# PeterFWS/Structure-PLP-SLAM

Measured on AMD Instinct MI355X. Metric: frames/sec ORB+LSD extract+match, 640x480 TUM-RGBD, 1/2/4/8 GPU, higher is better.
Workload: dtype u8

## Files before the change

include/plp_front.h:

```cpp
#ifndef PLP_FRONT_H
#define PLP_FRONT_H

#include <stddef.h>
#include <stdint.h>

#ifdef __cplusplus
extern "C" {
#endif

typedef enum plp_status {
    PLP_OK = 0,
    PLP_ERR_INVALID_ARG = 1,
    PLP_ERR_NO_DEVICE = 2,
    PLP_ERR_HIP = 3,
    PLP_ERR_CAPACITY = 4,
    PLP_ERR_OVERFLOW = 5,
    PLP_ERR_UNSUPPORTED = 6
} plp_status;

const char* plp_strerror(plp_status s);
const char* plp_last_error(void);
int plp_version(void);
int plp_device_count(void);

// ... 85 lines not shown

plp_status plp_line_extract(plp_line* ctx, const uint8_t* img, int32_t rows, int32_t cols, size_t step,
                            plp_keyline* kl, uint8_t* lbd, double* linefn, int32_t cap, int32_t* n_out);
plp_status plp_line_extract_batch_device(plp_line* ctx, const uint8_t* d_imgs, int32_t B, int32_t rows, int32_t cols,
                                         size_t step, size_t frame_stride, plp_keyline* d_kl, uint8_t* d_lbd,
                                         double* d_linefn, int32_t cap, int32_t* d_counts, void* hip_stream);
plp_status plp_line_last_batch_status(plp_line* ctx);
plp_status plp_line_set_profiling(plp_line* ctx, int32_t enable);
plp_status plp_line_get_stage_times(plp_line* ctx, double* ms9, int64_t* n_batches);
plp_status plp_line_set_grow_waves(plp_line* ctx, int32_t waves);
typedef enum plp_seed_order { PLP_SEED_ORDER_STABLE = 0, PLP_SEED_ORDER_LIBSTDCXX = 1 } plp_seed_order;
plp_status plp_line_set_seed_order(plp_line* ctx, int32_t order);
plp_status plp_line_get_seed_order(const plp_line* ctx, int32_t* order);
plp_status plp_line_trim(plp_line* ctx);

typedef enum plp_line_debug_id { PLP_LINE_DBG_SCALED = 0, PLP_LINE_DBG_ORDER = 1, PLP_LINE_DBG_RAW = 2, PLP_LINE_DBG_ALL_KL = 3,
                                 PLP_LINE_DBG_ALL_LBD = 4, PLP_LINE_DBG_SOBEL_DX = 5, PLP_LINE_DBG_SOBEL_DY = 6,
                                 PLP_LINE_DBG_GROW_STATS = 7  } plp_line_debug_id;
plp_status plp_line_debug_read(plp_line* ctx, plp_line_debug_id what, int32_t frame, void* dst, size_t dst_bytes, int64_t* n_out);
int32_t plp_model_index_sort_host(const int32_t* sizes, int32_t n, int32_t depth_limit, uint32_t* idx);
int32_t plp_model_quadtree_rank_sort_host(const uint32_t* keys, int32_t n, int32_t shift, uint32_t* perm);
int32_t plp_model_seed_introsort_host(uint32_t* entries, int64_t n, int32_t depth_limit, uint32_t skip_key);
plp_status plp_seed_introsort_debug(int32_t device, uint32_t* entries, int64_t n, int32_t depth_limit, uint32_t skip_key, int32_t variant, int32_t* n_live);
int32_t plp_model_sincos_host(const float* a, int64_t n, float* c, float* s, uint8_t* proven);
int32_t plp_model_null_vector4_host(const double* A, int32_t n, double* out_v, int32_t* out_sweeps);
plp_status plp_line_scaled_size(const plp_line* ctx, int32_t* rows, int32_t* cols);
plp_status plp_line_debug_grow_profile(plp_line* ctx, int64_t* out12);

typedef struct plp_keyline plp_keyline_fwd_;
typedef struct plp_matcher plp_matcher;
plp_status plp_matcher_create(int device, plp_matcher** out);
void plp_matcher_destroy(plp_matcher* ctx);

typedef enum plp_match_mode {
    PLP_MATCH_MODE_LANDMARKS = 0,
    PLP_MATCH_MODE_LAST_FRAME = 1,
    PLP_MATCH_MODE_BRUTE_FORCE = 2,
    PLP_MATCH_MODE_LANDMARKS_LINE = 3,
    PLP_MATCH_MODE_LAST_FRAME_LINE = 4,
    PLP_MATCH_MODE_BOW = 5,
    PLP_MATCH_MODE_FUSE = 6,
    PLP_MATCH_MODE_FUSE_LINE = 7,
    PLP_MATCH_MODE_TRIANGULATION = 8
} plp_match_mode;

#define PLP_MATCH_FLAG_NO_CHI2 1
// ... 1294 lines not shown
```

structure-plp-slam_amd/__init__.py:

```python
import ctypes as C
import math
import os
import pathlib
import subprocess

import numpy as np

from ._core import (LIB_PATH, PLP_ERR_CAPACITY, PLP_ERR_HIP, PLP_ERR_INVALID_ARG, PLP_ERR_NO_DEVICE, PLP_ERR_OVERFLOW, PLP_ERR_UNSUPPORTED, PLP_OK, PlpError,
                    ROOT, _API, _I32, _PKG, _SZ, _VP, _check, _lib, _p, api_symbols, build, lib)
from ._abi import *
from ._abi import _struct
from ._global_ba import (GLOBAL_BA_OUTPUTS, LOOP_BA_PROPAGATE_OUTPUTS, _chol_dense, _global_ba_host, _global_ba_kw, _loop_ba_propagate_host, global_bundle_adjuster,
                         loop_bundle_adjuster, model_chol_dense, model_global_ba, model_loop_ba_propagate)
from ._essential import (ESSENTIAL_OUTPUTS, _essential_ransac_host, essential_solver, model_essential_check, model_essential_draw, model_essential_fit,
                         model_essential_ransac)
from ._two_view import (TWO_VIEW_OUTPUTS, _two_view_pose_host, bearing_vector_initializer, model_check_pose, model_essential_decompose, model_two_view_pose,
                        two_view_args)
from ._line_update import (CORRECT_LINE_ERASED, CORRECT_LINE_NO_REF, CORRECT_LINE_NO_VERTEX, CORRECT_LINE_OK, LINE_MOVE_OUTPUTS, TRIM_DEPTH_POSITIVE, TRIM_INDEX_RANGE,
                           TRIM_MAX_CHANGE, TRIM_MAX_CHANGE_THR, TRIM_NO_REF, TRIM_NOT_OBSERVED, TRIM_OK, TRIM_OUTPUTS, TRIM_REJECTED, TRIM_SKIPPED,
                           correct_landmark_lines_args_c, line_update_entries, loop_ba_propagate_lines_args_c, model_correct_landmark_lines,
                           model_loop_ba_propagate_lines, model_trim_line_endpoints, trim_line_endpoints_args_c)
from ._marshal import _rows_u8, array_or_none, dev_ptr, dev_ptrs, host_ptr, host_ptrs, model_call, model_draw, out_arrays, set_outputs, stream_handle, wanted


# ... 2 lines not shown
    out = np.zeros(max(len(xys), 1), np.int32)
    m = lib().plp_model_quadtree_host(_p(xys), len(xys), level_w, level_h, quota, _p(out))
    return out[:m].copy()


def model_quadtree_rank_sort(keys, shift=0):
    k = np.ascontiguousarray(keys, np.uint32)
    perm = np.zeros(max(len(k), 1), np.uint32)
    assert lib().plp_model_quadtree_rank_sort_host(_p(k), len(k), int(shift), _p(perm)) == len(k)
    return perm[:len(k)].copy()


def model_seed_introsort(entries, depth_limit=-1, skip_key=0):
    e = np.ascontiguousarray(entries, np.uint32).copy()
    assert lib().plp_model_seed_introsort_host(_p(e), e.size, int(depth_limit), int(skip_key)) == 0
    return e


def seed_introsort_debug(entries, depth_limit=-1, skip_key=0, variant=0, device=0, return_live=False):
    e = np.ascontiguousarray(entries, np.uint32).copy()
    nl = C.c_int32(e.size)
    _check(lib().plp_seed_introsort_debug(int(device), _p(e), e.size, int(depth_limit), int(skip_key), int(variant), C.byref(nl)))
    return (e, nl.value) if return_live else e


def model_index_sort(sizes, depth_limit=-1):
    sz = np.ascontiguousarray(sizes, np.int32)
    idx = np.zeros(len(sz), np.uint32)
    assert lib().plp_model_index_sort_host(_p(sz), len(sz), int(depth_limit), _p(idx)) == len(sz)
    return idx


def model_sincos(a):
    a = np.ascontiguousarray(a, np.float32)
    c = np.zeros(a.shape, np.float32); s = np.zeros(a.shape, np.float32); ok = np.zeros(a.shape, np.uint8)
    lib().plp_model_sincos_host(_p(a), a.size, _p(c), _p(s), _p(ok))
    return c, s, ok.astype(bool)


def _landmark_geometry_host(call, lines, pose, feats, pos_w, ref_kf, obs_offsets, obs_kf, obs_idx, scale_factors, scale_factors_lsd, skip, counts,
                            out):
    po = np.ascontiguousarray(pose, np.float64).reshape(-1, 15)
    F = len(po)
    ft = np.ascontiguousarray(feats, KL_DTYPE if lines else KP_DTYPE).reshape(F, -1)
    M = ft.shape[1]
    pw = np.ascontiguousarray(pos_w, np.float64).reshape(-1, 6 if lines else 3)
# ... 2906 lines not shown
```

structure-plp-slam_amd/_core.py:

```python

import ctypes as C
import os
import pathlib
import subprocess


_PKG = pathlib.Path(__file__).resolve().parent
ROOT = _PKG.parent
LIB_PATH = pathlib.Path(os.environ["PLP_FRONT_LIB"]).resolve() if os.environ.get("PLP_FRONT_LIB") else _PKG / "libplp_front.so"


PLP_OK, PLP_ERR_INVALID_ARG, PLP_ERR_NO_DEVICE, PLP_ERR_HIP, PLP_ERR_CAPACITY, PLP_ERR_OVERFLOW, PLP_ERR_UNSUPPORTED = range(7)


class PlpError(RuntimeError):
    def __init__(self, status, detail):
        super().__init__(f"plp_front status {status}: {detail}")
        self.status = status


def build(verbose=False):
    r = subprocess.run(["make", "-j", str(min(8, os.cpu_count() or 1)), "-C", str(_PKG / "csrc")], capture_output=not verbose, text=True)
    if r.returncode != 0:
        raise RuntimeError("building libplp_front.so failed:\n" + (r.stdout or "") + (r.stderr or ""))
# ... 19 lines not shown
    ("plp_orb_last_batch_status", C.c_int, [_VP]),
    ("plp_orb_set_profiling", C.c_int, [_VP, _I32]),
    ("plp_orb_get_stage_times", C.c_int, [_VP, _VP, _VP]),
    ("plp_orb_pyramid_level_size", C.c_int, [_VP, _I32, _VP, _VP]),
    ("plp_orb_pyramid_host", C.c_int, [_VP, _I32, _I32, _VP, _SZ]),
    ("plp_orb_debug_read", C.c_int, [_VP, C.c_int, _I32, _I32, _VP, _SZ, _VP]),
    ("plp_model_quadtree_host", _I32, [_VP, _I32, _I32, _I32, C.c_uint32, _VP]),
    ("plp_model_quadtree_rank_sort_host", _I32, [_VP, _I32, _I32, _VP]),
    ("plp_model_sincos_host", _I32, [_VP, C.c_int64, _VP, _VP, _VP]),
    ("plp_model_index_sort_host", _I32, [_VP, _I32, _I32, _VP]),
    ("plp_model_null_vector4_host", _I32, [_VP, _I32, _VP, _VP]),
    ("plp_line_create", C.c_int, [C.c_int, _VP]),
    ("plp_line_destroy", None, [_VP]),
    ("plp_line_extract", C.c_int, [_VP, _VP, _I32, _I32, _SZ, _VP, _VP, _VP, _I32, _VP]),
    ("plp_line_extract_batch_device", C.c_int, [_VP, _VP, _I32, _I32, _I32, _SZ, _SZ, _VP, _VP, _VP, _I32, _VP, _VP]),
    ("plp_line_last_batch_status", C.c_int, [_VP]),
    ("plp_line_set_profiling", C.c_int, [_VP, _I32]),
    ("plp_line_set_grow_waves", C.c_int, [_VP, _I32]),
    ("plp_line_set_seed_order", C.c_int, [_VP, _I32]),
    ("plp_line_get_seed_order", C.c_int, [_VP, _VP]),
    ("plp_line_trim", C.c_int, [_VP]),
    ("plp_model_seed_introsort_host", _I32, [_VP, C.c_int64, _I32, C.c_uint32]),
    ("plp_seed_introsort_debug", C.c_int, [_I32, _VP, C.c_int64, _I32, C.c_uint32, _I32, _VP]),
    ("plp_line_get_stage_times", C.c_int, [_VP, _VP, _VP]),
    ("plp_line_debug_read", C.c_int, [_VP, C.c_int, _I32, _VP, _SZ, _VP]),
    ("plp_line_scaled_size", C.c_int, [_VP, _VP, _VP]),
    ("plp_line_debug_grow_profile", C.c_int, [_VP, _VP]),
    ("plp_matcher_create", C.c_int, [C.c_int, _VP]),
    ("plp_matcher_destroy", None, [_VP]),
    ("plp_match_device", C.c_int, [_VP, _VP, _VP]),
    ("plp_match_host", C.c_int, [_VP, _VP]),
    ("plp_match_debug_counters", C.c_int, [_VP, _VP]),
    ("plp_match_debug_plan", C.c_int, [_VP, _VP]),
    ("plp_match_area_host", C.c_int, [_VP, _VP, _VP, _I32, _VP, _VP, _I32, _VP, _VP, _I32, C.c_float, _I32, _VP, _VP]),
    ("plp_convert_to_grayscale_device", C.c_int, [_VP, _VP, _I32, _I32, C.c_size_t, C.c_size_t, _I32, _I32, _I32, _VP, C.c_size_t, C.c_size_t, _VP]),
    ("plp_convert_to_true_depth_device", C.c_int, [_VP, _VP, _I32, _I32, _I32, C.c_size_t, C.c_size_t, C.c_double, _I32, _VP, C.c_size_t, C.c_size_t, _VP]),
    ("plp_rectify_map_device", C.c_int, [_VP, _VP, _VP, _I32, _VP, _VP, _I32, _I32, _VP, _VP, C.c_size_t, _VP]),
    ("plp_rectify_map_fisheye_device", C.c_int, [_VP, _VP, _VP, _VP, _VP, _I32, _I32, _VP, _VP, C.c_size_t, _VP]),
    ("plp_remap_linear_device", C.c_int, [_VP, _VP, _I32, _I32, C.c_size_t, C.c_size_t, _VP, _VP, C.c_size_t, _I32, _I32, _I32, _VP, C.c_size_t, C.c_size_t, _VP]),
    ("plp_bow_vocab_create", C.c_int, [C.c_int, _VP, _VP]),
    ("plp_bow_vocab_destroy", None, [_VP]),
    ("plp_bow_transform_device", C.c_int, [_VP, _VP, _VP, _I32, _I32, _I32, _VP, _VP, _VP, _VP, _VP, _VP, _VP, _VP, _VP]),
    ("plp_bow_transform_host", C.c_int, [_VP, _VP, _I32, _I32, _VP, _VP, _VP, _VP, _VP, _VP, _VP, _VP]),
    ("plp_bow_query_device", C.c_int, [_VP, _VP, _VP]),
    ("plp_bow_query_host", C.c_int, [_VP, _VP]),
    ("plp_bow_score_pairs_device", C.c_int, [_VP, _VP, _VP]),
# ... 180 lines not shown
```

structure-plp-slam_amd/csrc/line_context.hip:

```cpp
#include <hip/hip_runtime.h>

#include <algorithm>
#include <cmath>
#include <cstring>
#include <mutex>
#include <vector>

#include "line_device.hpp"
#include "null4.hpp"
#include "seed_sort_model.hpp"
#include "sincos_ziv.hpp"
#include "plp_common.hpp"

using namespace plp;

struct plp_line {
    HostPinned pin;
    int device = 0;
    hipStream_t stream = nullptr;
    hipStream_t idle_stream = nullptr;
    int rows = 0, cols = 0, capB = 0;
    int grow_waves = 0;
    int seed_order = PLP_SEED_ORDER_LIBSTDCXX;
    bool mw_ok = false, seed_sort_ok = false;
// ... 412 lines not shown

int32_t plp_model_sincos_host(const float* a, int64_t n, float* c, float* s, uint8_t* proven) {
    int32_t n_proven = 0;
    for (int64_t i = 0; i < n; ++i) { proven[i] = plp::sincos_ziv(a[i], c + i, s + i) ? 1 : 0; n_proven += proven[i]; }
    return n_proven;
}

int32_t plp_model_null_vector4_host(const double* A, int32_t n, double* out_v, int32_t* out_sweeps) {
    if (!A || !out_v || n < 0) return -1;
    for (int32_t i = 0; i < n; ++i) {
        int sweeps = 0;
        plp::null_vector4(A + 16 * (size_t)i, out_v + 4 * (size_t)i, &sweeps);
        if (out_sweeps) out_sweeps[i] = sweeps;
    }
    return n;
}

int32_t plp_model_seed_introsort_host(uint32_t* entries, int64_t n, int32_t depth_limit, uint32_t skip_key) {
    if (!entries || n < 0 || n > (int64_t)kLsdMaxScaledPixels) return -1;
    plp::seedsort::introsort_loop_model(entries, (int)n, depth_limit, skip_key);
    return 0;
}

plp_status plp_seed_introsort_debug(int32_t device, uint32_t* entries, int64_t n, int32_t depth_limit, uint32_t skip_key, int32_t variant, int32_t* n_live) {
    if (!entries || n < 0 || n > (int64_t)kLsdMaxScaledPixels) return set_error(PLP_ERR_INVALID_ARG, "bad entries");
    int nd = 0;
    if (hipGetDeviceCount(&nd) != hipSuccess || nd == 0) return set_error(PLP_ERR_NO_DEVICE, "no HIP device visible");
    PLP_HIP(hipSetDevice(device));
    PLP_HIP(seed_sort_configure());
    if (depth_limit < 0) { int lg = 0; while ((2ll << lg) <= n) ++lg; depth_limit = 2 * lg; }
    DevBuf ent, ws, st;
    const int copies = std::max(1, std::min(4096, getenv("PLP_SEED_SORT_DBG_COPIES") ? atoi(getenv("PLP_SEED_SORT_DBG_COPIES")) : 1));
    PLP_HIP(ent.reserve((size_t)std::max<int64_t>(n, 1) * 4 * copies)); PLP_HIP(ws.reserve(seed_sort_ws_entries((size_t)n) * 4 * copies)); PLP_HIP(st.reserve(16));
    for (int k = 0; k < copies; ++k) PLP_HIP(hipMemcpy((uint32_t*)ent.p + (size_t)k * n, entries, (size_t)n * 4, hipMemcpyHostToDevice));
    PLP_HIP(hipMemset(st.p, 0, 16));
    DevBuf dbg;
    const char* dflag = getenv("PLP_SEED_SORT_DBG");
    if (dflag) { PLP_HIP(dbg.reserve(4 * (2 + 6 * 4000 + 48))); PLP_HIP(hipMemset(dbg.p, 0, 4 * (2 + 6 * 4000 + 48))); int f = atoi(dflag); PLP_HIP(hipMemcpy(dbg.p, &f, 4, hipMemcpyHostToDevice)); }
    launch_seed_sort_debug(nullptr, (uint32_t*)ent.p, (int)n, depth_limit, skip_key, (uint32_t*)ws.p, (int32_t*)st.p, dflag ? (int*)dbg.p : nullptr, variant, copies);
    PLP_HIP(hipGetLastError());
    PLP_HIP(hipDeviceSynchronize());
    int32_t s = 0;
    PLP_HIP(hipMemcpy(&s, st.p, 4, hipMemcpyDeviceToHost));
    PLP_HIP(hipMemcpy(entries, ent.p, (size_t)n * 4, hipMemcpyDeviceToHost));
    if (n_live) { uint32_t nl = (uint32_t)n; if (n > 16) PLP_HIP(hipMemcpy(&nl, ws.p, 4, hipMemcpyDeviceToHost)); *n_live = (int32_t)nl; }
    if (dflag && getenv("PLP_SEED_SORT_DBG_FILE")) {
// ... 10 lines not shown
```

structure-plp-slam_amd/csrc/line_device.hpp:

```cpp
#pragma once
#include <hip/hip_runtime.h>
#include <stdint.h>

#include "../../include/plp_front.h"

namespace plp {

constexpr int kMwHeap = 16384;
constexpr int kMwHeapBufs = 2;
constexpr int kMwMaxWaves = 8;
constexpr int kLsdMwMaxFrames = 256;
constexpr int kLineCap = 2048;
constexpr double kLsdNotDef = -1024.0;
constexpr int kLsdSeedPixBits = 20;
constexpr uint32_t kLsdSeedPixMask = (1u << kLsdSeedPixBits) - 1u;
constexpr size_t kLsdGrowLdsBytes = 66560;
constexpr size_t kLsdMaxScaledPixels = (kLsdGrowLdsBytes / 4 - 256) * 32 - 31;
static_assert(kLsdMaxScaledPixels <= (size_t)kLsdSeedPixMask + 1, "seed packing of k_lsd_order must hold every admitted pixel index");
static_assert(kLsdSeedPixBits + 10 <= 32, "10 bits of gradient bin above the pixel field");

struct alignas(16) LsdPix { float deg; uint32_t g2; float2 cs; };
__device__ __forceinline__ double pix_ang(const LsdPix& p) { return (double)p.deg * (3.14159265358979323846 / 180); }
__device__ __forceinline__ double pix_mod(const LsdPix& p) { return sqrt((double)p.g2 / 4.0); }

// ... 25 lines not shown
};

__host__ __device__ inline size_t dxy_frame_entries(int W, int H) { return (size_t)((W + 7) / 8) * ((H + 3) / 4) * 32; }
__host__ __device__ inline int dxy_index(int x, int y, int tiles_x) { return (((y >> 2) * tiles_x + (x >> 3)) << 5) + ((y & 3) << 3) + (x & 7); }

struct LsdParams {
    double prec, p, rho, density_th, scale;
    int n_bins, refine, min_reg_size;
    float min_length;
    float keep_length;
    float c_pass, c_fail;
    uint32_t g2_def_min;
    int seed_exact;
};
constexpr double kLsdAngleBand = 3.5e-4;
constexpr double kLsdBandMinPrec = 0.01, kLsdBandMaxPrec = 1.5;

struct ResizeExactTab { const int16_t *xo, *xc, *yo, *yc; };
struct BlurTapsN { int k[11]; };
struct LbdWeightsDev { float g[63], l[21], l2[21]; };

struct SeedSortBufs { uint32_t* ent; uint32_t* ws; size_t ws_stride; };
size_t seed_sort_ws_entries(size_t nv);
hipError_t seed_sort_configure();
void launch_seed_order_exact(hipStream_t st, const LinePlanes& P, const LsdParams& lp, int B, uint32_t* ent, uint32_t* ws, size_t ws_stride);
void launch_seed_sort_debug(hipStream_t st, uint32_t* ent, int n, int depth, uint32_t skip_key, uint32_t* ws, int32_t* status, int* dbg, int variant, int copies = 1);
hipError_t grow_mw_configure();
hipError_t grow_configure();

void launch_line_front(hipStream_t st, const LinePlanes& P, const LsdParams& lp, const ResizeExactTab& rt, const BlurTapsN& t11,
                       const BlurTapsN& t5, const LbdWeightsDev& w, plp_keyline* out_kl, uint8_t* out_lbd, double* out_fn, int cap,
                       int32_t* out_counts, int B, hipEvent_t* ev, int grow_waves, const SeedSortBufs* seed_exact, bool mw_ok);

}
```

structure-plp-slam_amd/csrc/seed_sort_impl.inc:

```
namespace SS_NS {


using seedsort::KeyDesc;
using seedsort::median3_pos;
using seedsort::select64;
using seedsort::select64_top;

constexpr int kSsWaves = SS_WAVES, kSsThreads = 64 * kSsWaves;
typedef uint16_t lrpos_t;
constexpr int kSsT = SS_T;

constexpr int kSsTask = kSsT < SS_TASK ? kSsT : SS_TASK;
constexpr int kSsSmall = 64;
constexpr int kSsSub = 256;
constexpr int kSubK = kSsSub / 64;
constexpr int kSsShift = seedsort::kKeyShift;
static_assert(kSsShift == kLsdSeedPixBits, "entry layout = the seed packing of k_lsd_order");
constexpr uint32_t kSsDefBit = 1u << 19;
static_assert(kLsdMaxScaledPixels <= (size_t)kSsDefBit, "pixel index below the defined bit");
constexpr int kSsQueue = kSsT <= 4096 ? 128 : 512, kSsSmallCap = kSsT <= 4096 ? 256 : 1536, kSsGStack = 64, kSsWStack = 8;
static_assert((kSsQueue & (kSsQueue - 1)) == 0 && kSsT / (kSsSub + 1) < kSsQueue && kSsT / 17 < kSsSmallCap && kSsT / (kSsTask + 1) < kSsWStack, "queue capacities");
constexpr int kSsChunksW = kSsT / 64 + 1;
constexpr int kSsMaxChunksG = (int)((kLsdMaxScaledPixels + 63) / 64) + 1;

struct SsCtl {
    int bc[8];
    int wsum[2][kSsWaves];
    int g_n; int g_first[kSsGStack], g_last[kSsGStack], g_depth[kSsGStack];
    int w_n; int w_first[kSsWStack], w_last[kSsWStack], w_depth[kSsWStack];
    int q_head, q_tail, q_pending, q_open, n_small, small_head, overflow;
    int n_live;
    long long t[24];
};

constexpr size_t kOffCtl = 0;
constexpr size_t kOffQ = (sizeof(SsCtl) + 7) / 8 * 8;
constexpr size_t kOffSmall = kOffQ + (size_t)kSsQueue * 8;
constexpr size_t kOffML = (kOffSmall + (size_t)kSsSmallCap * 4 + 7) / 8 * 8;
constexpr size_t kOffMR = kOffML + (size_t)kSsChunksW * 8;
constexpr size_t kOffPA = kOffMR + (size_t)kSsChunksW * 8;
constexpr size_t kOffPBx = kOffPA + (size_t)kSsChunksW * 4;
constexpr size_t kOffPBi = kOffPBx + (size_t)kSsChunksW * 4;
constexpr size_t kOffRpos = (kOffPBi + (size_t)kSsChunksW * 4 + 15) / 16 * 16;
constexpr size_t kOffWin = kOffRpos + ((size_t)(kSsT / 2 + 64) * sizeof(lrpos_t) + 15) / 16 * 16;
constexpr size_t kSsLdsBytes = kOffWin + (size_t)kSsT * 4 + 16;
static_assert(kOffRpos + (size_t)kSsMaxChunksG * 12 <= 160 * 1024 && kSsLdsBytes <= 160 * 1024, "LDS of the seed sort");

struct SsMem {
    uint32_t* a;
    void* rpos;
    uint32_t* xr;
    unsigned long long *mL, *mR;
    uint32_t *pA, *pBx, *pBi;
    size_t lds_bytes_g;
};

__device__ __forceinline__ int wave_incl_scan(int v, int lane) {
    v += __builtin_amdgcn_update_dpp(0, v, 0x111, 0xf, 0xf, false);
    v += __builtin_amdgcn_update_dpp(0, v, 0x112, 0xf, 0xf, false);
    v += __builtin_amdgcn_update_dpp(0, v, 0x114, 0xf, 0xf, false);
    v += __builtin_amdgcn_update_dpp(0, v, 0x118, 0xf, 0xf, false);
    const int t0 = __builtin_amdgcn_readlane(v, 15), t1 = __builtin_amdgcn_readlane(v, 31), t2 = __builtin_amdgcn_readlane(v, 47);
    return v + (lane >= 16 ? t0 : 0) + (lane >= 32 ? t1 : 0) + (lane >= 48 ? t2 : 0);
}
__device__ __forceinline__ int wave_max(int v) {
    v = max(v, __builtin_amdgcn_update_dpp(v, v, 0x128, 0xf, 0xf, false));
    v = max(v, __builtin_amdgcn_update_dpp(v, v, 0x124, 0xf, 0xf, false));
    v = max(v, __builtin_amdgcn_update_dpp(v, v, 0x122, 0xf, 0xf, false));
    v = max(v, __builtin_amdgcn_update_dpp(v, v, 0x121, 0xf, 0xf, false));
    return max(max(__builtin_amdgcn_readlane(v, 0), __builtin_amdgcn_readlane(v, 16)), max(__builtin_amdgcn_readlane(v, 32), __builtin_amdgcn_readlane(v, 48)));
}
__device__ __forceinline__ unsigned long long readlane64(unsigned long long v, int src) {
    const unsigned lo = (unsigned)__builtin_amdgcn_readlane((int)(unsigned)v, src), hi = (unsigned)__builtin_amdgcn_readlane((int)(unsigned)(v >> 32), src);
    return ((unsigned long long)hi << 32) | lo;
// ... 2 lines not shown
__device__ __forceinline__ int uni(int v) { return __builtin_amdgcn_readfirstlane(v); }
__device__ __forceinline__ unsigned long long bits_above(unsigned long long m, int lane) { return (m >> lane) >> 1; }
__device__ __forceinline__ int below_cnt(unsigned long long m) { return (int)__builtin_amdgcn_mbcnt_hi((unsigned)(m >> 32), __builtin_amdgcn_mbcnt_lo((unsigned)m, 0u)); }
__device__ __forceinline__ int above_cnt(unsigned long long m, int lane) { return __popcll(m) - below_cnt(m) - (int)((m >> lane) & 1ull); }

#define SS_PLAIN_BARRIER() wg_barrier()
template <bool G> __device__ __forceinline__ void ss_barrier() {
    if constexpr (G) wg_barrier_after_global_stores(); else wg_barrier();
}

template <class Pred> __device__ __forceinline__ int wave_count_prefix(int nch, int lane, Pred pred) {
    int lo = 0, hi = nch;
    while (lo < hi) {
        const int step = (hi - lo + 63) >> 6, c = lo + lane * step;
        const int t = __popcll(__ballot(c < hi && pred(c)));
        if (t == 0) { hi = lo; break; }
        const int nlo = lo + (t - 1) * step + 1;
        hi = min(hi, lo + t * step);
        lo = nlo;
    }
    return lo;
}

template <bool G, bool LM = false> __device__ __forceinline__ int wg_partition(const SsMem& M, SsCtl* ctl, int first, int last, uint32_t skip_key, bool prof = false) {
    long long tp0 = prof ? clock64() : 0;
    auto plap = [&](int k) { if (prof && threadIdx.x == 0) { const long long t1 = clock64(); ctl->t[(G ? 16 : 10) + k] += t1 - tp0; tp0 = t1; } };
    using rpos_t = typename std::conditional<G, uint32_t, lrpos_t>::type;
    constexpr int U = G ? 8 : 4, UA = G ? 16 : 4;
    [[maybe_unused]] rpos_t* rpos = (rpos_t*)M.rpos + (G ? 0 : (first >> 1));
    uint32_t* a = M.a;
    const int tid = threadIdx.x, lane = tid & 63, wv = uni(tid >> 6);
    first = uni(first); last = uni(last);
    const int p0 = first + 1, np = last - p0, nch = (np + 63) >> 6, mid = first + (last - first) / 2;
    SsMem Q = M;
    if constexpr (G) {
        const int nchp = (nch + 2) & ~1;
        Q.pA = M.pA; Q.pBx = M.pA + nchp; Q.pBi = M.pA + 2 * nchp;
        if constexpr (LM) { Q.mL = (unsigned long long*)(M.pA + 3 * nchp); Q.mR = Q.mL + nch; }
    }
    const uint32_t e0 = a[first], ea = a[p0], eb = a[mid], ec = a[last - 1];
    const int m3 = median3_pos(ea >> kSsShift, eb >> kSsShift, ec >> kSsShift, p0, mid, last - 1);
    const uint32_t em = m3 == p0 ? ea : (m3 == mid ? eb : ec), pk = em >> kSsShift;
    for (int c0 = wv * UA; c0 < nch; c0 += kSsWaves * UA) {
        uint32_t e[UA];
#pragma unroll
        for (int u = 0; u < UA; ++u) {
            const int pos = p0 + ((c0 + u) << 6) + lane;
            e[u] = pos < last ? a[pos] : 0u;
        }
#pragma unroll
        for (int u = 0; u < UA; ++u) {
            const int c = c0 + u, pos = p0 + (c << 6) + lane;
            if (c >= nch) break;
            const bool valid = pos < last;
            const uint32_t k = (pos == m3 ? e0 : e[u]) >> kSsShift;
            const unsigned long long mL = __ballot(valid && k <= pk), mR = __ballot(valid && k >= pk);
            if (lane == 0) { Q.mL[c] = mL; Q.mR[c] = mR; Q.pA[c] = (uint32_t)__popcll(mL); Q.pBx[c] = (uint32_t)__popcll(mR); }
        }
    }
    ss_barrier<G>();
    plap(0);
// ... 38 lines not shown
                const int c = wave_count_prefix(nch, lane, [&](int c) { return (int)Q.pA[c] <= m; }) - 1;
                Lm = p0 + (c << 6) + select64(Q.mL[c], m - (int)Q.pA[c]);
            }
            const int c = wave_count_prefix(nch, lane, [&](int c) { return (int)Q.pBx[c] > m - 1; });
            cut = min(Lm, p0 + (c << 6) + select64_top(Q.mR[c], m - 1 - (int)Q.pBx[c]));
        }
        const int totR = uni(ctl->bc[4]);
        const bool sane = m >= 0 && m <= min(totL, totR) && cut > first && cut <= last;
        if (lane == 0) {
            if (sane) { a[first] = em; a[m3] = e0; ctl->bc[0] = m; ctl->bc[1] = cut; }
            else { ctl->bc[0] = 0; ctl->bc[1] = last; if (!ctl->overflow) { ctl->overflow = 1; ctl->bc[6] = m; ctl->bc[7] = cut; } }
            ctl->bc[3] = (int)pk;
            if constexpr (G) {
                const bool dead = sane && pk < skip_key && last == ctl->n_live;
                ctl->bc[5] = dead ? 1 : 0;
                if (dead) ctl->n_live = cut;
            }
        }
    }
    ss_barrier<G>();
    plap(2);
    const int m = uni(ctl->bc[0]), cut = uni(ctl->bc[1]);
    if constexpr (G) {
        uint32_t* xl = (uint32_t*)Q.rpos; uint32_t* xr = Q.xr;
        const bool dead = uni(ctl->bc[5]) != 0;
        auto left_chunks = [&](auto&& body) {
            for (int c0 = wv * U; c0 < nch; c0 += kSsWaves * U) {
                if (uni((int)Q.pA[c0]) >= m) break;
                unsigned long long mk[U]; int r0[U];
#pragma unroll
                for (int u = 0; u < U; ++u) { const int c = c0 + u; mk[u] = c < nch ? Q.mL[c] : 0ull; r0[u] = c < nch ? (int)Q.pA[c] : m; }
                int rank[U];
#pragma unroll
                for (int u = 0; u < U; ++u) { const int r = r0[u] + below_cnt(mk[u]); rank[u] = (((mk[u] >> lane) & 1ull) && r < m) ? r : -1; }
                body(c0, rank);
            }
        };
        auto right_chunks = [&](auto&& body) {
            for (int c0 = nch - 1 - wv * U; c0 >= 0; c0 -= kSsWaves * U) {
                if (uni((int)Q.pBx[c0]) >= m) break;
                unsigned long long mk[U]; int r0[U];
#pragma unroll
                for (int u = 0; u < U; ++u) { const int c = c0 - u; mk[u] = c >= 0 ? Q.mR[c] : 0ull; r0[u] = c >= 0 ? (int)Q.pBx[c] : m; }
                int rank[U];
#pragma unroll
                for (int u = 0; u < U; ++u) { const int r = r0[u] + above_cnt(mk[u], lane); rank[u] = (((mk[u] >> lane) & 1ull) && r < m) ? r : -1; }
                body(c0, rank);
            }
        };
        if (!dead) left_chunks([&](int c0, const int (&rank)[U]) {
            uint32_t v[U];
#pragma unroll
            for (int u = 0; u < U; ++u) if (rank[u] >= 0) v[u] = a[p0 + ((c0 + u) << 6) + lane];
#pragma unroll
            for (int u = 0; u < U; ++u) if (rank[u] >= 0) xl[rank[u]] = v[u];
        });
        right_chunks([&](int c0, const int (&rank)[U]) {
            uint32_t v[U];
#pragma unroll
            for (int u = 0; u < U; ++u) if (rank[u] >= 0) v[u] = a[p0 + ((c0 - u) << 6) + lane];
#pragma unroll
            for (int u = 0; u < U; ++u) if (rank[u] >= 0) xr[rank[u]] = v[u];
        });
        ss_barrier<G>();
        plap(3);
        left_chunks([&](int c0, const int (&rank)[U]) {
            uint32_t v[U];
#pragma unroll
            for (int u = 0; u < U; ++u) if (rank[u] >= 0) v[u] = xr[rank[u]];
#pragma unroll
            for (int u = 0; u < U; ++u) if (rank[u] >= 0) a[p0 + ((c0 + u) << 6) + lane] = v[u];
        });
        if (!dead) right_chunks([&](int c0, const int (&rank)[U]) {
            uint32_t v[U];
#pragma unroll
            for (int u = 0; u < U; ++u) if (rank[u] >= 0) v[u] = xl[rank[u]];
#pragma unroll
            for (int u = 0; u < U; ++u) if (rank[u] >= 0) a[p0 + ((c0 - u) << 6) + lane] = v[u];
        });
        ss_barrier<G>();
        plap(4);
    } else {
    for (int c0 = nch - 1 - wv * U; c0 >= 0; c0 -= kSsWaves * U) {
        if (uni((int)Q.pBx[c0]) >= m) break;
        unsigned long long mR[U]; int bx[U];
#pragma unroll
        for (int u = 0; u < U; ++u) { const int c = c0 - u; mR[u] = c >= 0 ? Q.mR[c] : 0ull; bx[u] = c >= 0 ? (int)Q.pBx[c] : m; }
#pragma unroll
        for (int u = 0; u < U; ++u)
            if ((mR[u] >> lane) & 1ull) {
                const int rank = bx[u] + above_cnt(mR[u], lane);
                if (rank < m) rpos[rank] = (rpos_t)(p0 + ((c0 - u) << 6) + lane);
            }
    }
    ss_barrier<G>();
    plap(3);
    for (int c0 = wv * U; c0 < nch; c0 += kSsWaves * U) {
        if (uni((int)Q.pA[c0]) >= m) break;
        int i[U], j[U]; uint32_t vi[U], vj[U];
#pragma unroll
        for (int u = 0; u < U; ++u) {
            const int c = c0 + u;
            i[u] = -1;
            if (c < nch) {
// ... 477 lines not shown
    lap(3);
    const int ns = uni(ctl->overflow) ? 0 : min(uni(ctl->n_small), kSsSmallCap);
    while (true) {
        int i = ticket;
        ticket = -1;
        if (i < 0) { if (lane == 0) i = lds_add(&ctl->small_head, 1); i = __builtin_amdgcn_readfirstlane(i); }
        if (i >= ns) break;
        const uint32_t r = (uint32_t)__builtin_amdgcn_readfirstlane((int)W.small[i]);
        const int first = (int)(r & 0xffffu);
        wave_sub_sort(W.win, W.rpos, first, first + (int)((r >> 16) & 0xffu) + 1, (int)(r >> 24), lane, W.skip_key, ctl, W.dbg != nullptr);
    }
    wg_barrier();
    lap(4);
    for (int i = tid; i < n; i += kSsThreads) ent[gfirst + i] = W.win[i];
    wg_barrier();
    lap(5);
    if (W.dbg && tid == 0) ctl->t[6] += 1;
}

__device__ __forceinline__ void seed_introsort_loop(uint32_t* ent, int n, int depth, uint32_t skip_key, uint32_t* ws, unsigned char* lds, int32_t* status, int* dbg = nullptr) {
    const int tid = threadIdx.x;
    SsCtl* ctl = (SsCtl*)(lds + kOffCtl);
    SsWin W{(uint32_t*)(lds + kOffWin), (lrpos_t*)(lds + kOffRpos), (unsigned long long*)(lds + kOffQ), (uint32_t*)(lds + kOffSmall), ctl, dbg, skip_key};
    const SsMem ML{W.win, W.rpos, nullptr, (unsigned long long*)(lds + kOffML), (unsigned long long*)(lds + kOffMR), (uint32_t*)(lds + kOffPA), (uint32_t*)(lds + kOffPBx), (uint32_t*)(lds + kOffPBi), 0};
    const int nchg = (n + 63) / 64 + 1;
    const size_t xlen = ((size_t)n / 2 + 64 + 1) & ~(size_t)1;
    uint32_t* g_xl = ws + 2;
    unsigned long long* g_mL = (unsigned long long*)(ws + 2 + 2 * xlen);
    const size_t lds_total = kSsLdsBytes > kOffRpos + 12 * ((size_t)(n + 63) / 64 + 1) + 16 ? kSsLdsBytes : kOffRpos + 12 * ((size_t)(n + 63) / 64 + 1) + 16;
    const SsMem MG{ent, g_xl, g_xl + xlen, g_mL, g_mL + nchg, (uint32_t*)(lds + kOffRpos), nullptr, nullptr, lds_total - kOffRpos - 16};
    if (tid == 0) { ctl->g_n = 1; ctl->g_first[0] = 0; ctl->g_last[0] = n; ctl->g_depth[0] = depth; ctl->overflow = 0; ctl->n_live = n; for (int k = 0; k < 24; ++k) ctl->t[k] = 0; }
    while (true) {
        ss_barrier<true>();
        const int sn = uni(ctl->g_n);
        if (sn == 0) break;
        if (uni(ctl->overflow)) break;
        const int first = uni(ctl->g_first[sn - 1]), last = uni(ctl->g_last[sn - 1]), d = uni(ctl->g_depth[sn - 1]);
        wg_barrier();
        if (tid == 0) ctl->g_n = sn - 1;
        if (last - first <= 16) continue;
        if (last - first <= kSsT) { window_process(ent, first, last, d, W, ML); continue; }
        if (d == 0) {
            if (tid == 0) libstdcxx::heap_sort(ent, first, last, KeyDesc());
            continue;
        }
        const long long tg = dbg ? clock64() : 0;
        const int nch_p = (last - first - 1 + 63) >> 6;
        const bool lm = (size_t)((nch_p + 2) & ~1) * 12 + (size_t)nch_p * 16 <= MG.lds_bytes_g;
        const int cut = lm ? wg_partition<true, true>(MG, ctl, first, last, skip_key, dbg != nullptr) : wg_partition<true, false>(MG, ctl, first, last, skip_key, dbg != nullptr);
        if (dbg && tid == 0) { ctl->t[0] += clock64() - tg; ctl->t[7] += 1; }
        if (tid == 0) {
            int i = ctl->g_n;
            if (i + 2 <= kSsGStack) {
                ctl->g_first[i] = first; ctl->g_last[i] = cut; ctl->g_depth[i] = d - 1; ++i;
                if ((uint32_t)ctl->bc[3] >= skip_key) { ctl->g_first[i] = cut; ctl->g_last[i] = last; ctl->g_depth[i] = d - 1; ++i; }
                ctl->g_n = i;
            } else ctl->overflow = 8;
        }
    }
    if (tid == 0) { ws[0] = (uint32_t)(ctl->overflow ? n : ctl->n_live); if (ctl->overflow) { if (atomicOr(status, 32) & 32) {} else { status[1] = ctl->overflow; status[2] = (int32_t)blockIdx.x; status[3] = ctl->overflow == 9 ? ctl->bc[7] : ctl->bc[6]; } } }
    if (dbg && tid == 0) for (int k = 0; k < 24; ++k) { dbg[2 + 6 * 4000 + 2 * k] = (int)(ctl->t[k] & 0xffffffff); dbg[2 + 6 * 4000 + 2 * k + 1] = (int)(ctl->t[k] >> 32); }
}


inline size_t lds_bytes(size_t nv) { return std::max(kSsLdsBytes, kOffRpos + 12 * ((nv + 63) / 64 + 1) + 16); }

__global__ __launch_bounds__(kSsThreads, SS_MINW) void k_lsd_seed_sort(LinePlanes P, LsdParams lp, int n_grad_blocks, uint32_t* ent_all, uint32_t* ws_all, size_t ws_stride) {
    extern __shared__ __attribute__((aligned(16))) unsigned char ss_lds[];
    const int b = blockIdx.x, tid = threadIdx.x, lane = tid & 63, wv = uni(tid >> 6);
    const int n = P.sw * P.sh, nv = (P.sw - 1) * (P.sh - 1);
    SsCtl* ctl = (SsCtl*)(ss_lds + kOffCtl);
    uint32_t mx = 0;
// ... 31 lines not shown
```

structure-plp-slam_amd/csrc/seed_sort_kernels.hip:

```cpp
#include <hip/hip_runtime.h>

#include <algorithm>
#include <type_traits>

#include "line_device.hpp"
#include "plp_barrier.hpp"
#include "seed_sort_model.hpp"

namespace plp {

#define SS_NS ss_thr
#define SS_WAVES 4
#define SS_T 4096
#define SS_MINW 4
#define SS_TASK 4096
#include "seed_sort_impl.inc"
#undef SS_NS
#undef SS_WAVES
#undef SS_T
#undef SS_MINW
#undef SS_TASK
#define SS_NS ss_lat
#define SS_WAVES 16
#define SS_T 24576
#define SS_MINW 1
#define SS_TASK 4096
#include "seed_sort_impl.inc"
#undef SS_NS
#undef SS_WAVES
#undef SS_T
#undef SS_MINW
#undef SS_TASK

constexpr int kSsLatMaxFrames = 256;

size_t seed_sort_ws_entries(size_t nv) { return 2 + 2 * ((nv / 2 + 64 + 1) & ~(size_t)1) + 2 * 2 * ((nv + 63) / 64 + 1); }

__global__ __launch_bounds__(256) void k_lsd_order_entries(LinePlanes P, const uint32_t* __restrict__ ent_all, const uint32_t* __restrict__ ws_all, size_t ws_stride) {
    __shared__ uint32_t cnt[4][1024];
    __shared__ uint32_t s_wsum[4];
    const int b = blockIdx.x, tid = threadIdx.x, lane = tid & 63, q = tid >> 6;
    const int nv_all = (P.sw - 1) * (P.sh - 1);
    const int nv = min(nv_all, (int)__builtin_amdgcn_readfirstlane((int)ws_all[(size_t)b * ws_stride]));
    for (int i = tid; i < 4096; i += 256) (&cnt[0][0])[i] = 0;
    wg_barrier();
    const uint32_t* ent = ent_all + (size_t)b * nv_all;
    uint32_t* order = P.order + (size_t)b * nv_all;
    const int ngroups = (nv + 63) / 64, gper = (ngroups + 3) / 4, g0 = q * gper, g1 = min(ngroups, g0 + gper);
    uint32_t* comp = P.reg + (size_t)b * P.reg_frame_stride + (size_t)g0 * 64;
    int ncomp = 0;
    for (int gb = g0; gb < g1; gb += 4) {
        uint32_t v4[4];
#pragma unroll
        for (int u = 0; u < 4; ++u) {
            const int i = (gb + u) * 64 + lane;
            v4[u] = (gb + u < g1 && i < nv) ? ent[i] : 0u;
        }
#pragma unroll
        for (int u = 0; u < 4; ++u) {
// ... 54 lines not shown
            if (valid && (peers & ((1ull << lane) - 1ull)) == 0) cnt[q][v] += (uint32_t)__popcll(peers);
            __builtin_amdgcn_wave_barrier();
        }
    }
}

void launch_seed_order_exact(hipStream_t st, const LinePlanes& P, const LsdParams& lp, int B, uint32_t* ent, uint32_t* ws, size_t ws_stride) {
    const int n = P.sw * P.sh;
    const size_t nv = (size_t)(P.sw - 1) * (P.sh - 1);
    if (B <= kSsLatMaxFrames) hipLaunchKernelGGL(ss_lat::k_lsd_seed_sort, dim3(B), dim3(ss_lat::kSsThreads), ss_lat::lds_bytes(nv), st, P, lp, (n + 255) / 256, ent, ws, ws_stride);
    else hipLaunchKernelGGL(ss_thr::k_lsd_seed_sort, dim3(B), dim3(ss_thr::kSsThreads), ss_thr::lds_bytes(nv), st, P, lp, (n + 255) / 256, ent, ws, ws_stride);
    hipLaunchKernelGGL(k_lsd_order_entries, dim3(B), dim3(256), 0, st, P, (const uint32_t*)ent, (const uint32_t*)ws, ws_stride);
}
hipError_t seed_sort_configure() {
    const void* fns[4] = {reinterpret_cast<const void*>(ss_thr::k_lsd_seed_sort), reinterpret_cast<const void*>(ss_thr::k_seed_sort_debug),
                          reinterpret_cast<const void*>(ss_lat::k_lsd_seed_sort), reinterpret_cast<const void*>(ss_lat::k_seed_sort_debug)};
    const size_t bytes[4] = {ss_thr::lds_bytes(kLsdMaxScaledPixels), ss_thr::lds_bytes(kLsdMaxScaledPixels), ss_lat::lds_bytes(kLsdMaxScaledPixels), ss_lat::lds_bytes(kLsdMaxScaledPixels)};
    for (int i = 0; i < 4; ++i) {
        const hipError_t e = hipFuncSetAttribute(fns[i], hipFuncAttributeMaxDynamicSharedMemorySize, (int)bytes[i]);
        if (e != hipSuccess) return e;
    }
    return hipSuccess;
}
void launch_seed_sort_debug(hipStream_t st, uint32_t* ent, int n, int depth, uint32_t skip_key, uint32_t* ws, int32_t* status, int* dbg, int variant, int copies) {
    const size_t ws_stride = seed_sort_ws_entries((size_t)n);
    if (variant) hipLaunchKernelGGL(ss_lat::k_seed_sort_debug, dim3(copies), dim3(ss_lat::kSsThreads), ss_lat::lds_bytes((size_t)n), st, ent, n, depth, skip_key, ws, ws_stride, status, dbg);
    else hipLaunchKernelGGL(ss_thr::k_seed_sort_debug, dim3(copies), dim3(ss_thr::kSsThreads), ss_thr::lds_bytes((size_t)n), st, ent, n, depth, skip_key, ws, ws_stride, status, dbg);
}

}
```

Before: 99260.

## Exchange global-partition elements through LDS tiles instead of global scratch buffers

The global-level partition in the seed sort used to scatter misplaced left and right elements into two global-memory scratch arrays and then gather them back. It now walks the exchange in rank windows sized to the free LDS, staging each window in LDS tiles with two workgroup barriers per window. This removes the large global scratch from the workspace and the global round trip, at the cost of extra barriers and ballot-based chunk-range scans per window. A small query entry point is added to report the tile size.

```diff
diff --git a/include/plp_front.h b/include/plp_front.h
--- a/include/plp_front.h
+++ b/include/plp_front.h
@@ -131,6 +131,7 @@
 int32_t plp_model_quadtree_rank_sort_host(const uint32_t* keys, int32_t n, int32_t shift, uint32_t* perm);
 int32_t plp_model_seed_introsort_host(uint32_t* entries, int64_t n, int32_t depth_limit, uint32_t skip_key);
 plp_status plp_seed_introsort_debug(int32_t device, uint32_t* entries, int64_t n, int32_t depth_limit, uint32_t skip_key, int32_t variant, int32_t* n_live);
+int32_t plp_seed_sort_tile_ranks(int64_t n_frame, int64_t n_segment, int32_t variant, int32_t* masks_in_lds);
 int32_t plp_model_sincos_host(const float* a, int64_t n, float* c, float* s, uint8_t* proven);
 int32_t plp_model_null_vector4_host(const double* A, int32_t n, double* out_v, int32_t* out_sweeps);
 plp_status plp_line_scaled_size(const plp_line* ctx, int32_t* rows, int32_t* cols);
diff --git a/structure-plp-slam_amd/__init__.py b/structure-plp-slam_amd/__init__.py
--- a/structure-plp-slam_amd/__init__.py
+++ b/structure-plp-slam_amd/__init__.py
@@ -48,6 +48,14 @@
     nl = C.c_int32(e.size)
     _check(lib().plp_seed_introsort_debug(int(device), _p(e), e.size, int(depth_limit), int(skip_key), int(variant), C.byref(nl)))
     return (e, nl.value) if return_live else e
+
+
+def seed_sort_tile_ranks(n_frame, n_segment=None, variant=0, return_masks=False):
+    lm = C.c_int32(0)
+    r = lib().plp_seed_sort_tile_ranks(int(n_frame), int(n_frame if n_segment is None else n_segment), int(variant), C.byref(lm))
+    if r < 0:
+        raise ValueError("bad arguments")
+    return (r, bool(lm.value)) if return_masks else r
 
 
 def model_index_sort(sizes, depth_limit=-1):
diff --git a/structure-plp-slam_amd/_core.py b/structure-plp-slam_amd/_core.py
--- a/structure-plp-slam_amd/_core.py
+++ b/structure-plp-slam_amd/_core.py
@@ -65,6 +65,7 @@
     ("plp_line_trim", C.c_int, [_VP]),
     ("plp_model_seed_introsort_host", _I32, [_VP, C.c_int64, _I32, C.c_uint32]),
     ("plp_seed_introsort_debug", C.c_int, [_I32, _VP, C.c_int64, _I32, C.c_uint32, _I32, _VP]),
+    ("plp_seed_sort_tile_ranks", _I32, [C.c_int64, C.c_int64, _I32, _VP]),
     ("plp_line_get_stage_times", C.c_int, [_VP, _VP, _VP]),
     ("plp_line_debug_read", C.c_int, [_VP, C.c_int, _I32, _VP, _SZ, _VP]),
     ("plp_line_scaled_size", C.c_int, [_VP, _VP, _VP]),
diff --git a/structure-plp-slam_amd/csrc/line_context.hip b/structure-plp-slam_amd/csrc/line_context.hip
--- a/structure-plp-slam_amd/csrc/line_context.hip
+++ b/structure-plp-slam_amd/csrc/line_context.hip
@@ -458,6 +458,14 @@
     return 0;
 }
 
+int32_t plp_seed_sort_tile_ranks(int64_t n_frame, int64_t n_segment, int32_t variant, int32_t* masks_in_lds) {
+    if (n_frame < 0 || n_frame > (int64_t)kLsdMaxScaledPixels || n_segment < 2 || n_segment > n_frame || variant < 0 || variant > 1) return -1;
+    int lm = 0;
+    const int r = seed_sort_tile_ranks((size_t)n_frame, (size_t)n_segment, variant, &lm);
+    if (masks_in_lds) *masks_in_lds = lm;
+    return r;
+}
+
 plp_status plp_seed_introsort_debug(int32_t device, uint32_t* entries, int64_t n, int32_t depth_limit, uint32_t skip_key, int32_t variant, int32_t* n_live) {
     if (!entries || n < 0 || n > (int64_t)kLsdMaxScaledPixels) return set_error(PLP_ERR_INVALID_ARG, "bad entries");
     int nd = 0;
diff --git a/structure-plp-slam_amd/csrc/line_device.hpp b/structure-plp-slam_amd/csrc/line_device.hpp
--- a/structure-plp-slam_amd/csrc/line_device.hpp
+++ b/structure-plp-slam_amd/csrc/line_device.hpp
@@ -71,6 +71,7 @@
 
 struct SeedSortBufs { uint32_t* ent; uint32_t* ws; size_t ws_stride; };
 size_t seed_sort_ws_entries(size_t nv);
+int seed_sort_tile_ranks(size_t nv, size_t n_seg, int variant, int* lm);
 hipError_t seed_sort_configure();
 void launch_seed_order_exact(hipStream_t st, const LinePlanes& P, const LsdParams& lp, int B, uint32_t* ent, uint32_t* ws, size_t ws_stride);
 void launch_seed_sort_debug(hipStream_t st, uint32_t* ent, int n, int depth, uint32_t skip_key, uint32_t* ws, int32_t* status, int* dbg, int variant, int copies = 1);
diff --git a/structure-plp-slam_amd/csrc/seed_sort_impl.inc b/structure-plp-slam_amd/csrc/seed_sort_impl.inc
--- a/structure-plp-slam_amd/csrc/seed_sort_impl.inc
+++ b/structure-plp-slam_amd/csrc/seed_sort_impl.inc
@@ -46,10 +46,20 @@
 constexpr size_t kSsLdsBytes = kOffWin + (size_t)kSsT * 4 + 16;
 static_assert(kOffRpos + (size_t)kSsMaxChunksG * 12 <= 160 * 1024 && kSsLdsBytes <= 160 * 1024, "LDS of the seed sort");
 
+constexpr int kSsTileMin = 512;
+__host__ __device__ constexpr size_t ss_tile_off(int nch, bool lm) { return (size_t)((nch + 2) & ~1) * 8 + (lm ? (size_t)nch * 16 : 0); }
+__host__ __device__ inline int ss_tile_plan(int n_seg, size_t area, bool* lm) {
+    const int nch = (n_seg - 1 + 63) >> 6;
+    const size_t offL = ss_tile_off(nch, true), offN = ss_tile_off(nch, false);
+    const size_t rL = area > offL ? (area - offL) / 8 : 0, rN = area > offN ? (area - offN) / 8 : 0;
+    *lm = rL >= (size_t)kSsTileMin && offL + (size_t)((nch + 2) & ~1) * 4 <= area;
+    return (int)(*lm ? rL : rN);
+}
+static_assert((kSsLdsBytes - kOffRpos - 16) / 24 >= 64 + 2, "every global partition has an exchange tile");
+
 struct SsMem {
     uint32_t* a;
     void* rpos;
-    uint32_t* xr;
     unsigned long long *mL, *mR;
     uint32_t *pA, *pBx, *pBi;
     size_t lds_bytes_g;
@@ -98,12 +108,13 @@
     return lo;
 }
 
-template <bool G, bool LM = false> __device__ __forceinline__ int wg_partition(const SsMem& M, SsCtl* ctl, int first, int last, uint32_t skip_key, bool prof = false) {
+template <bool G, bool LM = false> __device__ __forceinline__ int wg_partition(const SsMem& M, SsCtl* ctl, int first, int last, uint32_t skip_key, bool prof = false, int tile_ranks = 0) {
     long long tp0 = prof ? clock64() : 0;
     auto plap = [&](int k) { if (prof && threadIdx.x == 0) { const long long t1 = clock64(); ctl->t[(G ? 16 : 10) + k] += t1 - tp0; tp0 = t1; } };
-    using rpos_t = typename std::conditional<G, uint32_t, lrpos_t>::type;
-    constexpr int U = G ? 8 : 4, UA = G ? 16 : 4;
-    [[maybe_unused]] rpos_t* rpos = (rpos_t*)M.rpos + (G ? 0 : (first >> 1));
+    using rpos_t = lrpos_t;
+    [[maybe_unused]] constexpr int U = 4;
+    constexpr int UA = G ? 16 : 4;
+    [[maybe_unused]] rpos_t* rpos = G ? nullptr : (rpos_t*)M.rpos + (first >> 1);
     uint32_t* a = M.a;
     const int tid = threadIdx.x, lane = tid & 63, wv = uni(tid >> 6);
     first = uni(first); last = uni(last);
@@ -111,8 +122,9 @@
     SsMem Q = M;
     if constexpr (G) {
         const int nchp = (nch + 2) & ~1;
-        Q.pA = M.pA; Q.pBx = M.pA + nchp; Q.pBi = M.pA + 2 * nchp;
-        if constexpr (LM) { Q.mL = (unsigned long long*)(M.pA + 3 * nchp); Q.mR = Q.mL + nch; }
+        Q.pA = M.pA; Q.pBx = M.pA + nchp;
+        if constexpr (LM) { Q.mL = (unsigned long long*)(M.pA + 2 * nchp); Q.mR = Q.mL + nch; }
+        Q.pBi = (uint32_t*)((unsigned char*)M.pA + ss_tile_off(nch, LM));
     }
     const uint32_t e0 = a[first], ea = a[p0], eb = a[mid], ec = a[last - 1];
     const int m3 = median3_pos(ea >> kSsShift, eb >> kSsShift, ec >> kSsShift, p0, mid, last - 1);
@@ -197,64 +209,55 @@
     plap(2);
     const int m = uni(ctl->bc[0]), cut = uni(ctl->bc[1]);
     if constexpr (G) {
-        uint32_t* xl = (uint32_t*)Q.rpos; uint32_t* xr = Q.xr;
+        constexpr int UT = 4;
+        const int R = uni(tile_ranks);
+        uint32_t* tileL = Q.pBi; uint32_t* tileR = tileL + R;
         const bool dead = uni(ctl->bc[5]) != 0;
-        auto left_chunks = [&](auto&& body) {
-            for (int c0 = wv * U; c0 < nch; c0 += kSsWaves * U) {
-                if (uni((int)Q.pA[c0]) >= m) break;
-                unsigned long long mk[U]; int r0[U];
-#pragma unroll
-                for (int u = 0; u < U; ++u) { const int c = c0 + u; mk[u] = c < nch ? Q.mL[c] : 0ull; r0[u] = c < nch ? (int)Q.pA[c] : m; }
-                int rank[U];
-#pragma unroll
-                for (int u = 0; u < U; ++u) { const int r = r0[u] + below_cnt(mk[u]); rank[u] = (((mk[u] >> lane) & 1ull) && r < m) ? r : -1; }
-                body(c0, rank);
-            }
-        };
-        auto right_chunks = [&](auto&& body) {
-            for (int c0 = nch - 1 - wv * U; c0 >= 0; c0 -= kSsWaves * U) {
-                if (uni((int)Q.pBx[c0]) >= m) break;
-                unsigned long long mk[U]; int r0[U];
-#pragma unroll
-                for (int u = 0; u < U; ++u) { const int c = c0 - u; mk[u] = c >= 0 ? Q.mR[c] : 0ull; r0[u] = c >= 0 ? (int)Q.pBx[c] : m; }
-                int rank[U];
-#pragma unroll
-                for (int u = 0; u < U; ++u) { const int r = r0[u] + above_cnt(mk[u], lane); rank[u] = (((mk[u] >> lane) & 1ull) && r < m) ? r : -1; }
-                body(c0, rank);
-            }
-        };
-        if (!dead) left_chunks([&](int c0, const int (&rank)[U]) {
-            uint32_t v[U];
-#pragma unroll
-            for (int u = 0; u < U; ++u) if (rank[u] >= 0) v[u] = a[p0 + ((c0 + u) << 6) + lane];
-#pragma unroll
-            for (int u = 0; u < U; ++u) if (rank[u] >= 0) xl[rank[u]] = v[u];
-        });
-        right_chunks([&](int c0, const int (&rank)[U]) {
-            uint32_t v[U];
-#pragma unroll
-            for (int u = 0; u < U; ++u) if (rank[u] >= 0) v[u] = a[p0 + ((c0 - u) << 6) + lane];
-#pragma unroll
-            for (int u = 0; u < U; ++u) if (rank[u] >= 0) xr[rank[u]] = v[u];
-        });
+        const int wr = kSsWaves - 1 - wv;
+        int cL = 0, cR = nch - 1;
+        for (int r0 = 0; r0 < m; r0 += R) {
+            const int r1 = min(r0 + R, m);
+            int cLe = cL, cRe = cR;
+            while (true) { const int c = cLe + lane, k = __popcll(__ballot(c < nch && (int)Q.pA[c] < r1)); cLe += k; if (k < 64) break; }
+            while (true) { const int c = cRe - lane, k = __popcll(__ballot(c >= 0 && (int)Q.pBx[c] < r1)); cRe -= k; if (k < 64) break; }
+            cLe = uni(cLe); cRe = uni(cRe);
+            auto pass = [&](auto is_left, auto is_put) {
+                constexpr bool LEFT = decltype(is_left)::value, PUT = decltype(is_put)::value;
+                uint32_t* mine = LEFT ? tileL : tileR; const uint32_t* theirs = LEFT ? tileR : tileL;
+                const unsigned long long* msk = LEFT ? Q.mL : Q.mR; const uint32_t* pre = LEFT ? Q.pA : Q.pBx;
+                const int cb = LEFT ? cL : cR, nj = LEFT ? cLe - cL : cR - cRe;
+                for (int j0 = (LEFT ? wv : wr) * UT; j0 < nj; j0 += kSsWaves * UT) {
+                    [[maybe_unused]] uint32_t e[UT];
+                    if constexpr (PUT) {
+#pragma unroll
+                        for (int u = 0; u < UT; ++u) {
+                            const int pos = p0 + ((LEFT ? cb + j0 + u : cb - j0 - u) << 6) + lane;
+                            e[u] = (j0 + u < nj && pos < last) ? a[pos] : 0u;
+                        }
+                    }
+#pragma unroll
+                    for (int u = 0; u < UT; ++u) {
+                        if (j0 + u >= nj) break;
+                        const int c = LEFT ? cb + j0 + u : cb - j0 - u;
+                        const unsigned long long mk = msk[c];
+                        const int r = (int)pre[c] + (LEFT ? below_cnt(mk) : above_cnt(mk, lane));
+                        if (((mk >> lane) & 1ull) && r >= r0 && r < r1) {
+                            if constexpr (PUT) mine[r - r0] = e[u];
+                            else a[p0 + (c << 6) + lane] = theirs[r - r0];
+                        }
+                    }
+                }
+            };
+            if (!dead) pass(std::true_type{}, std::true_type{});
+            pass(std::false_type{}, std::true_type{});
+            wg_barrier();
+            pass(std::true_type{}, std::false_type{});
+            if (!dead) pass(std::false_type{}, std::false_type{});
+            wg_barrier();
+            cL = cLe - 1; cR = cRe + 1;
+        }
         ss_barrier<G>();
         plap(3);
-        left_chunks([&](int c0, const int (&rank)[U]) {
-            uint32_t v[U];
-#pragma unroll
-            for (int u = 0; u < U; ++u) if (rank[u] >= 0) v[u] = xr[rank[u]];
-#pragma unroll
-            for (int u = 0; u < U; ++u) if (rank[u] >= 0) a[p0 + ((c0 + u) << 6) + lane] = v[u];
-        });
-        if (!dead) right_chunks([&](int c0, const int (&rank)[U]) {
-            uint32_t v[U];
-#pragma unroll
-            for (int u = 0; u < U; ++u) if (rank[u] >= 0) v[u] = xl[rank[u]];
-#pragma unroll
-            for (int u = 0; u < U; ++u) if (rank[u] >= 0) a[p0 + ((c0 - u) << 6) + lane] = v[u];
-        });
-        ss_barrier<G>();
-        plap(4);
     } else {
     for (int c0 = nch - 1 - wv * U; c0 >= 0; c0 -= kSsWaves * U) {
         if (uni((int)Q.pBx[c0]) >= m) break;
@@ -778,13 +781,11 @@
     const int tid = threadIdx.x;
     SsCtl* ctl = (SsCtl*)(lds + kOffCtl);
     SsWin W{(uint32_t*)(lds + kOffWin), (lrpos_t*)(lds + kOffRpos), (unsigned long long*)(lds + kOffQ), (uint32_t*)(lds + kOffSmall), ctl, dbg, skip_key};
-    const SsMem ML{W.win, W.rpos, nullptr, (unsigned long long*)(lds + kOffML), (unsigned long long*)(lds + kOffMR), (uint32_t*)(lds + kOffPA), (uint32_t*)(lds + kOffPBx), (uint32_t*)(lds + kOffPBi), 0};
+    const SsMem ML{W.win, W.rpos, (unsigned long long*)(lds + kOffML), (unsigned long long*)(lds + kOffMR), (uint32_t*)(lds + kOffPA), (uint32_t*)(lds + kOffPBx), (uint32_t*)(lds + kOffPBi), 0};
     const int nchg = (n + 63) / 64 + 1;
-    const size_t xlen = ((size_t)n / 2 + 64 + 1) & ~(size_t)1;
-    uint32_t* g_xl = ws + 2;
-    unsigned long long* g_mL = (unsigned long long*)(ws + 2 + 2 * xlen);
+    unsigned long long* g_mL = (unsigned long long*)(ws + 2);
     const size_t lds_total = kSsLdsBytes > kOffRpos + 12 * ((size_t)(n + 63) / 64 + 1) + 16 ? kSsLdsBytes : kOffRpos + 12 * ((size_t)(n + 63) / 64 + 1) + 16;
-    const SsMem MG{ent, g_xl, g_xl + xlen, g_mL, g_mL + nchg, (uint32_t*)(lds + kOffRpos), nullptr, nullptr, lds_total - kOffRpos - 16};
+    const SsMem MG{ent, nullptr, g_mL, g_mL + nchg, (uint32_t*)(lds + kOffRpos), nullptr, nullptr, lds_total - kOffRpos - 16};
     if (tid == 0) { ctl->g_n = 1; ctl->g_first[0] = 0; ctl->g_last[0] = n; ctl->g_depth[0] = depth; ctl->overflow = 0; ctl->n_live = n; for (int k = 0; k < 24; ++k) ctl->t[k] = 0; }
     while (true) {
         ss_barrier<true>();
@@ -801,9 +802,10 @@
             continue;
         }
         const long long tg = dbg ? clock64() : 0;
-        const int nch_p = (last - first - 1 + 63) >> 6;
-        const bool lm = (size_t)((nch_p + 2) & ~1) * 12 + (size_t)nch_p * 16 <= MG.lds_bytes_g;
-        const int cut = lm ? wg_partition<true, true>(MG, ctl, first, last, skip_key, dbg != nullptr) : wg_partition<true, false>(MG, ctl, first, last, skip_key, dbg != nullptr);
+        bool lm = false;
+        const int tile = uni(ss_tile_plan(last - first, MG.lds_bytes_g, &lm));
+        if (tile < 1) { if (tid == 0) ctl->overflow = 10; continue; }
+        const int cut = lm ? wg_partition<true, true>(MG, ctl, first, last, skip_key, dbg != nullptr, tile) : wg_partition<true, false>(MG, ctl, first, last, skip_key, dbg != nullptr, tile);
         if (dbg && tid == 0) { ctl->t[0] += clock64() - tg; ctl->t[7] += 1; }
         if (tid == 0) {
             int i = ctl->g_n;
diff --git a/structure-plp-slam_amd/csrc/seed_sort_kernels.hip b/structure-plp-slam_amd/csrc/seed_sort_kernels.hip
--- a/structure-plp-slam_amd/csrc/seed_sort_kernels.hip
+++ b/structure-plp-slam_amd/csrc/seed_sort_kernels.hip
@@ -34,7 +34,7 @@
 
 constexpr int kSsLatMaxFrames = 256;
 
-size_t seed_sort_ws_entries(size_t nv) { return 2 + 2 * ((nv / 2 + 64 + 1) & ~(size_t)1) + 2 * 2 * ((nv + 63) / 64 + 1); }
+size_t seed_sort_ws_entries(size_t nv) { return 2 + 2 * 2 * ((nv + 63) / 64 + 1); }
 
 __global__ __launch_bounds__(256) void k_lsd_order_entries(LinePlanes P, const uint32_t* __restrict__ ent_all, const uint32_t* __restrict__ ws_all, size_t ws_stride) {
     __shared__ uint32_t cnt[4][1024];
@@ -135,6 +135,12 @@
     }
     return hipSuccess;
 }
+int seed_sort_tile_ranks(size_t nv, size_t n_seg, int variant, int* lm) {
+    bool l = false;
+    const int r = variant ? ss_lat::ss_tile_plan((int)n_seg, ss_lat::lds_bytes(nv) - ss_lat::kOffRpos - 16, &l) : ss_thr::ss_tile_plan((int)n_seg, ss_thr::lds_bytes(nv) - ss_thr::kOffRpos - 16, &l);
+    if (lm) *lm = l ? 1 : 0;
+    return r;
+}
 void launch_seed_sort_debug(hipStream_t st, uint32_t* ent, int n, int depth, uint32_t skip_key, uint32_t* ws, int32_t* status, int* dbg, int variant, int copies) {
     const size_t ws_stride = seed_sort_ws_entries((size_t)n);
     if (variant) hipLaunchKernelGGL(ss_lat::k_seed_sort_debug, dim3(copies), dim3(ss_lat::kSsThreads), ss_lat::lds_bytes((size_t)n), st, ent, n, depth, skip_key, ws, ws_stride, status, dbg);
```

After: 101,600, median of 6. 1.02x the previous value.
